# GEOS-ESM/QuickChem

Hardware: AMD Instinct MI355X
Metric: OH gridcells/sec (XGBoost predict), C360 L72 batch (higher is better)
Workload: dtype f32

## Files before the change

### include/ohxgb.h

```cpp
#ifndef OHXGB_H_
#define OHXGB_H_

#include <stdint.h>

#ifdef __cplusplus
extern "C" {
#endif

typedef void* DMatrixHandle;
typedef void* BoosterHandle;
typedef uint64_t bst_ulong;


const char* XGBGetLastError(void);

int XGDMatrixCreateFromMat(const float* data, bst_ulong nrow, bst_ulong ncol, float missing, DMatrixHandle* out);

int XGDMatrixFree(DMatrixHandle handle);

int XGDMatrixNumRow(DMatrixHandle handle, bst_ulong* out);
int XGDMatrixNumCol(DMatrixHandle handle, bst_ulong* out);

int XGDMatrixSaveBinary(DMatrixHandle handle, const char* fname, int silent);
int XGDMatrixCreateFromFile(const char* fname, int silent, DMatrixHandle* out);
// ... 73 lines not shown
  float *ndwet;
  int32_t *k1, *k2;
  float *diag_pl_bst, *diag_tauclwdn, *diag_tauclidn, *diag_taucliup, *diag_tauclwup;
  float *diag_aodup, *diag_aoddn, *diag_aod, *diag_strato3;
} OHXRun1Args;

int OHXBoosterRun1(BoosterHandle handle, const OHXRun1Args* args);
int OHXBoosterRun1Device(BoosterHandle handle, const OHXRun1Args* args, void* stream);

int OHXOHPostProcess(int im, int jm, int km, float avogad, float runiv, float epsilon, const float* ple_mod,
                     const float* t_mod, const float* q_mod, const float* tropp_mod, const float* default_oh,
                     const float* oh_ml, float* oh, float* ndwet);
int OHXOHPostProcessDevice(int im, int jm, int km, float avogad, float runiv, float epsilon, const float* d_ple_mod,
                           const float* d_t_mod, const float* d_q_mod, const float* d_tropp_mod,
                           const float* d_default_oh, const float* d_oh_ml, float* d_oh, float* d_ndwet, void* stream);

int OHXJulianDay(int nymd, int* jday);
int OHXSolarGeometry(int jday, const float* lats, const float* lons, int im, int jm, float degrees_to_radians,
                     float radians_to_degrees, float* lat_deg, float* sza_noon);
int OHXSolarGeometryDevice(int jday, const float* d_lats, const float* d_lons, int im, int jm, float degrees_to_radians,
                           float radians_to_degrees, float* d_lat_deg, float* d_sza_noon, void* stream);

int OHXBoosterGetInfo(BoosterHandle handle, bst_ulong info[8]);
int OHXBoosterGetNumGroups(BoosterHandle handle, bst_ulong* out);
int OHXBoosterGetNumCategoricalSplits(BoosterHandle handle, bst_ulong* out);
int OHXBoosterKernelSymbol(BoosterHandle handle, bst_ulong ncol, const char** out);
int OHXBoosterKernelSymbolRows(BoosterHandle handle, DMatrixHandle dmat, const char** out);
int OHXBoosterRingReruns(BoosterHandle handle, void* stream, bst_ulong* out);
int OHXBoosterCopyEngineChoice(BoosterHandle handle, int* choice, unsigned* trials, unsigned* picked_dma);

typedef void* OHXCommHandle;
#define OHX_UNIQUE_ID_BYTES 128
int OHXCommGetUniqueId(void* id);
int OHXCommInitRank(const void* id, int nranks, int rank, OHXCommHandle* out);
int OHXCommFree(OHXCommHandle comm);
int OHXCommInfo(int* rccl_version);
int OHXShardRows(bst_ulong nrows_total, int nranks, int rank, bst_ulong* row0, bst_ulong* nrows);
int OHXAllGatherOH(OHXCommHandle comm, const float* d_shard, bst_ulong nrows_local, bst_ulong nrows_total,
                   float* d_full, void* stream);

int OHXUnregisterHost(const void* array);

int OHXReleaseScratch(void);

#ifdef __cplusplus
}
// ... 3 lines not shown
```

### quickchem_amd/capi.py

```python
from __future__ import annotations

import ctypes as C
import os
from typing import Optional, Sequence

import numpy as np

_HERE = os.path.dirname(os.path.abspath(__file__))
LIB_PATH = os.path.join(_HERE, "lib", "libohxgb.so")
RING_ROUNDS_DEFAULT = 64
RING_ROUNDS_NO_GRID = 16
RING_ROUNDS_PERMUTED = 4

ABI_SYMBOLS = [
    "XGBGetLastError", "XGDMatrixCreateFromMat", "XGDMatrixFree", "XGDMatrixNumRow", "XGDMatrixNumCol",
    "XGDMatrixSaveBinary", "XGDMatrixCreateFromFile", "XGBoosterCreate", "XGBoosterFree", "XGBoosterLoadModel",
    "XGBoosterSaveModel", "XGBoosterLoadModelFromBuffer", "XGBoosterPredict", "XGBoosterSetParam",
    "OHXDeviceCount", "OHXDMatrixCreateFromDevice", "OHXDMatrixSetGrid", "OHXDMatrixGetGrid", "OHXDMatrixInferGrid", "OHXBoosterPredictDevice", "OHXBoosterCheck",
    "OHXBoosterPredictContribs", "OHXBoosterPredictContribsDevice",
    "OHXBoosterPredictInteractions", "OHXBoosterPredictInteractionsDevice",
    "OHXBoosterPredictContribsFields", "OHXBoosterPredictContribsFieldsDevice",
    "OHXBoosterPredictFields", "OHXBoosterPredictFieldsDevice", "OHXBoosterRun1", "OHXBoosterRun1Device", "OHXOHPostProcess", "OHXOHPostProcessDevice",
    "OHXJulianDay", "OHXSolarGeometry", "OHXSolarGeometryDevice", "OHXBoosterGetInfo", "OHXBoosterGetNumGroups", "OHXBoosterGetNumCategoricalSplits", "OHXBoosterKernelSymbol", "OHXBoosterKernelSymbolRows",
    "OHXBoosterRingReruns", "OHXBoosterCopyEngineChoice", "OHXUnregisterHost", "OHXReleaseScratch",
    "OHXCommGetUniqueId", "OHXCommInitRank", "OHXCommFree", "OHXCommInfo", "OHXShardRows", "OHXAllGatherOH",
]
REFERENCE_BOUND_SYMBOLS = [
    "XGBoosterLoadModel", "XGBoosterSaveModel", "XGDMatrixSaveBinary", "XGDMatrixFree", "XGDMatrixCreateFromFile",
    "XGBoosterPredict", "XGBoosterCreate", "XGDMatrixCreateFromMat", "XGDMatrixNumRow", "XGDMatrixNumCol",
    "XGBoosterFree",
]


class OhxError(RuntimeError):
    pass


class OHXRun1Args(C.Structure):
    _P = C.c_void_p
    _fields_ = ([("im", C.c_int32), ("jm", C.c_int32), ("km", C.c_int32), ("dynamic_k_range", C.c_int32),
                 ("tropp_min", C.c_float), ("ohscale", C.c_float), ("missing", C.c_float),
                 ("avogad", C.c_float), ("runiv", C.c_float), ("epsilon", C.c_float)] +
                [(n, C.c_void_p) for n in ("ple_mod", "t_mod", "q_mod", "tropp_mod", "ple_bst", "zle_bst", "tauclw",
                                           "taucli")] +
                [("scacoef", C.c_void_p * 7)] +
                [(n, C.c_void_p) for n in ("gmito3", "gmitto3", "lat_deg", "t_bst", "no2", "o3", "ch4", "co", "isop",
# ... 51 lines not shown
    lib.OHXDMatrixInferGrid.argtypes = [vp, vp, C.POINTER(i32)]
    lib.OHXBoosterPredictDevice.argtypes = [vp, vp, i32, C.c_uint, vp, vp]
    lib.OHXBoosterCheck.argtypes = [vp, vp]
    lib.OHXBoosterPredictContribs.argtypes = [vp, vp, i32, C.c_uint, C.POINTER(u64), C.POINTER(C.POINTER(f32))]
    lib.OHXBoosterPredictContribsDevice.argtypes = [vp, vp, i32, C.c_uint, vp, vp]
    lib.OHXBoosterPredictInteractions.argtypes = [vp, vp, i32, C.c_uint, C.POINTER(u64), C.POINTER(C.POINTER(f32))]
    lib.OHXBoosterPredictInteractionsDevice.argtypes = [vp, vp, i32, C.c_uint, vp, vp]
    lib.OHXBoosterPredictContribsFields.argtypes = [vp, C.POINTER(vp), C.POINTER(C.c_int32), i32, i32, i32, i32, i32,
                                                    i32, i32, f32, i32, C.c_uint, C.POINTER(vp)]
    lib.OHXBoosterPredictContribsFieldsDevice.argtypes = [vp, C.POINTER(vp), C.POINTER(C.c_int32), i32, i32, i32, i32,
                                                          i32, i32, i32, f32, i32, C.c_uint, C.POINTER(vp), vp]
    lib.OHXBoosterPredictFields.argtypes = [vp, C.POINTER(vp), C.POINTER(C.c_int32), i32, i32, i32, i32, i32, i32, i32,
                                            f32, i32, f32, vp, vp]
    lib.OHXBoosterPredictFieldsDevice.argtypes = [vp, C.POINTER(vp), C.POINTER(C.c_int32), i32, i32, i32, i32, i32,
                                                  i32, i32, f32, i32, f32, vp, vp, vp]
    lib.OHXBoosterRun1.argtypes = [vp, C.POINTER(OHXRun1Args)]
    lib.OHXBoosterRun1Device.argtypes = [vp, C.POINTER(OHXRun1Args), vp]
    lib.OHXOHPostProcess.argtypes = [i32, i32, i32, f32, f32, f32] + [vp] * 8
    lib.OHXOHPostProcessDevice.argtypes = [i32, i32, i32, f32, f32, f32] + [vp] * 9
    lib.OHXJulianDay.argtypes = [i32, C.POINTER(i32)]
    lib.OHXSolarGeometry.argtypes = [i32, vp, vp, i32, i32, f32, f32, vp, vp]
    lib.OHXSolarGeometryDevice.argtypes = [i32, vp, vp, i32, i32, f32, f32, vp, vp, vp]
    lib.OHXBoosterGetInfo.argtypes = [vp, C.POINTER(u64)]
    lib.OHXBoosterGetNumGroups.argtypes = [vp, C.POINTER(u64)]
    lib.OHXBoosterGetNumCategoricalSplits.argtypes = [vp, C.POINTER(u64)]
    lib.OHXBoosterKernelSymbol.argtypes = [vp, u64, C.POINTER(C.c_char_p)]
    lib.OHXBoosterKernelSymbolRows.argtypes = [vp, vp, C.POINTER(C.c_char_p)]
    lib.OHXBoosterRingReruns.argtypes = [vp, vp, C.POINTER(u64)]
    lib.OHXBoosterCopyEngineChoice.argtypes = [vp, C.POINTER(C.c_int), C.POINTER(C.c_uint), C.POINTER(C.c_uint)]
    lib.OHXUnregisterHost.argtypes = [vp]
    lib.OHXReleaseScratch.argtypes = []
    lib.OHXCommGetUniqueId.argtypes = [vp]
    lib.OHXCommInitRank.argtypes = [vp, i32, i32, C.POINTER(vp)]
    lib.OHXCommFree.argtypes = [vp]
    lib.OHXCommInfo.argtypes = [C.POINTER(i32)]
    lib.OHXShardRows.argtypes = [u64, i32, i32, C.POINTER(u64), C.POINTER(u64)]
    lib.OHXAllGatherOH.argtypes = [vp, vp, u64, u64, vp, vp]
    if path == LIB_PATH:
        _lib = lib
    return lib


def check(lib: C.CDLL, rc: int) -> None:
    if rc != 0:
        raise OhxError(lib.XGBGetLastError().decode("utf-8", "replace"))

# ... 269 lines not shown
        if want_diag:
            for name in RUN1_DIAG_3D:
                diag[name] = np.zeros(im * jm * km, dtype=np.float32)
                setattr(args, name, diag[name].ctypes.data)
            diag["diag_strato3"] = np.zeros(im * jm, dtype=np.float32)
            args.diag_strato3 = diag["diag_strato3"].ctypes.data
        return {"args": args, "keep": keep, "oh": oh, "boost": boost, "ndwet": ndwet, "k1": k1, "k2": k2, "diag": diag,
                "shape": (im, jm, km)}

    def run1_call(self, call: dict) -> dict:
        im, jm, km = call["shape"]
        check(self.lib, self.lib.OHXBoosterRun1(self.handle, C.byref(call["args"])))
        unflat = lambda a: None if a is None else a.reshape(km, jm, im).transpose(2, 1, 0)
        out = {"oh": unflat(call["oh"]), "oh_boost": unflat(call["boost"]), "ndwet": unflat(call["ndwet"]),
               "k1": call["k1"].value, "k2": call["k2"].value}
        for name, a in call["diag"].items():
            out[name] = a.reshape(jm, im).T if name == "diag_strato3" else unflat(a)
        return out

    def run1(self, state: dict, **kw) -> dict:
        return self.run1_call(self.run1_prepare(state, **kw))

    def info(self) -> dict:
        arr = (C.c_uint64 * 8)()
        check(self.lib, self.lib.OHXBoosterGetInfo(self.handle, arr))
        keys = ["num_trees", "num_nodes", "num_slots", "node_bytes", "max_depth", "num_feature", "packed",
                "gathers_per_wave"]
        return {k: int(arr[i]) for i, k in enumerate(keys)}

    def ring_reruns(self, stream: int = 0) -> int:
        out = C.c_uint64()
        check(self.lib, self.lib.OHXBoosterRingReruns(self.handle, stream, C.byref(out)))
        return int(out.value)

    def copy_engine_choice(self):
        c, t, d = C.c_int(), C.c_uint(), C.c_uint()
        check(self.lib, self.lib.OHXBoosterCopyEngineChoice(self.handle, C.byref(c), C.byref(t), C.byref(d)))
        return int(c.value), int(t.value), int(d.value)

    def kernel_symbol(self, ncol: int) -> str:
        out = C.c_char_p()
        check(self.lib, self.lib.OHXBoosterKernelSymbol(self.handle, ncol, C.byref(out)))
        return out.value.decode()

    def kernel_symbols_for(self, dmat) -> str:
        out = C.c_char_p()
        check(self.lib, self.lib.OHXBoosterKernelSymbolRows(self.handle, dmat.handle, C.byref(out)))
        return out.value.decode()

    def fields_kernel_symbol(self, nrow: int = 1 << 30) -> str:
# ... 87 lines not shown
```

### quickchem_amd/csrc/capi.cpp

```cpp
#include <hip/hip_runtime_api.h>

#include <algorithm>
#include <cmath>
#include <cstdio>
#include <cstdlib>
#include <cstring>
#include <fstream>
#include <memory>
#include <atomic>
#include <chrono>
#include <mutex>
#include <unordered_map>
#include <sstream>
#include <string>
#include <unordered_set>
#include <vector>

#include "../../include/ohxgb.h"
#include "categorical.hpp"
#include "contribs.hpp"
#include "flatten.hpp"
#include "forest.hpp"
#include "groups.hpp"
#include "kernels.hpp"
// ... 465 lines not shown
  ~BoosterObj() {
    for (hipEvent_t e : {run1_fork, run1_slab, run1_join, run1_clear})
      if (e) (void)hipEventDestroy(e);
    for (hipEvent_t e : run1_prep) (void)hipEventDestroy(e);
    for (hipEvent_t e : run1_walk) (void)hipEventDestroy(e);
    for (hipEvent_t e : run1_feed_events) (void)hipEventDestroy(e);
    if (train.side) (void)hipStreamDestroy(train.side);
    if (train.fork) (void)hipEventDestroy(train.fork);
    if (train.join) (void)hipEventDestroy(train.join);
    if (cluster_done) (void)hipEventDestroy(cluster_done);
    if (defer_seen) (void)hipEventDestroy(defer_seen);
  }
  TrainStreams train;
  Forest forest;
  uint32_t num_groups = 1;
  Forest grouped;
  std::vector<uint32_t> group_begin;
  std::vector<uint32_t> flat_file_index;
  const Forest& flat() const { return num_groups >= 2 ? grouped : forest; }
  bool loaded = false;
  float margin_base = 0.0f;
  std::string margin_error;
  LayoutParams layout;
  std::string kernel_name = "auto";
  int device_pref = -1;
  LaunchTuning tune;
  bool uploaded = false;
  DeviceInfo dev;
  Placement placement;
  bool packed_ok = false;
  DevBuf<PackedNode> d_packed;
  DevBuf<WideNode> d_wide;
  DevBuf<SuperNode> d_super;
  DevBuf<SuperTreeHead> d_super_heads;
  bool super_ok = false;
  uint64_t super_slots = 0;
  uint64_t super_gathers[3] = {0, 0, 0};
  double super_mean_steps = 0.0;
  std::string symbol;
  DevBuf<uint32_t> d_roots;
  DevBuf<uint32_t> d_flags;
  uint32_t ring_reruns_seen = 0;
  DevBuf<float> d_leaves;
  DevBuf<uint32_t> d_defer;
  PinnedBuf<uint32_t> h_defer_count;
  PinnedBuf<uint32_t> h_flags;
  hipEvent_t defer_seen = nullptr;
  bool defer_pending = false;
  uint64_t defer_last_nrow = 0;
  bool defer_too_many = false;
  DevBuf<float> d_pred;
  PinnedBuf<float> h_pred;
  DevBuf<float> d_planes, d_gleaf;
  DevBuf<uint32_t> d_flat_of_file;
  hipStream_t s_copy = nullptr, s_exec = nullptr;
  hipEvent_t run1_fork = nullptr, run1_slab = nullptr, run1_join = nullptr, run1_clear = nullptr;
  std::vector<hipEvent_t> run1_prep, run1_walk, run1_feed_events;
  struct CopyEngineTrial {
    size_t vol = 0;
// ... 129 lines not shown

void ensure_uploaded(BoosterObj& b) {
  if (!b.loaded) throw OhxError("the booster holds no model: call XGBoosterLoadModel first");
  if (b.uploaded) {
    HIP_CHECK(hipSetDevice(b.dev.ordinal));
    return;
  }
  b.dev = use_device(b.device_pref);
  const Forest& flat = b.flat();
  b.placement = place_forest(flat, b.layout);
  b.packed_ok = packed_format_fits(flat, b.placement);
  b.d_roots.upload(b.placement.roots);
  if (b.num_cat != 0) {
    CatForest cf = emit_cat(flat, b.placement);
    b.cat_word_count = cf.words.size();
    b.cat_inline_sets = cf.inline_sets;
    b.cat_word_sets = cf.word_sets;
    if (cf.words.empty()) cf.words.push_back(0u);
    b.d_cat_nodes.upload(cf.nodes);
    b.d_cat_words.upload(cf.words);
    b.d_cat_orig.upload(cf.orig_id);
  } else if (wants_super(b.kernel_name)) {
    SuperForest sf;
    b.super_ok = emit_super(flat, &sf) && sf.nodes.size() * sizeof(SuperNode) < 0xFFFFFFF0ull;
    if (b.super_ok) {
      b.super_slots = sf.nodes.size();
      b.super_gathers[0] = count_super_gathers(sf, 0);
      b.super_gathers[1] = count_super_gathers(sf, 1);
      b.super_gathers[2] = count_super_gathers(sf, 2);
      b.super_mean_steps = mean_super_steps(sf);
      b.d_super.upload(sf.nodes);
      b.d_super_heads.upload(sf.heads);
    }
  }
  if (b.num_cat == 0 && b.packed_ok && !(b.super_ok && wants_super(b.kernel_name))) {
    std::vector<PackedNode> packed = emit_packed(flat, b.placement, nullptr);
    b.d_packed.upload(packed);
  }
  if (b.num_cat == 0 && pick_kernel(b) == KernelKind::Wide) ensure_wide(b);
  b.d_flags.ensure(3);
  {
    LibStreams& ls = lib_streams(b.dev.ordinal);
    b.s_exec = ls.exec;
    b.s_copy = ls.copy;
  }
  HIP_CHECK(hipMemsetAsync(b.d_flags.p, 0, 3 * sizeof(uint32_t), b.s_exec));
  HIP_CHECK(hipStreamSynchronize(b.s_exec));
  b.ring_reruns_seen = 0;
  ensure_train_stream(b);
  b.uploaded = true;
}

void ensure_train_stream(BoosterObj& b) {
  b.tune.train = nullptr;
// ... 1024 lines not shown
  }
  if (n == "ohx_register_host" && handle == nullptr) {
    g_host_registry.on.store(atoi(value) != 0);
    if (atoi(value) == 0) g_host_registry.release_all();
    return 0;
  }
  BoosterObj* b = as_booster(handle);
  if (n == "ohx_kernel") {
    if (v != "auto" && v != "wide" && v != "packed1" && v != "packed2" && v != "packed4" && v != "super1" &&
        v != "super2" && v != "super3" && v != "super4" && v != "ring")
      throw OhxError("ohx_kernel must be one of auto, wide, packed1, packed2, packed4, super1 .. super4, ring");
    if (v != b->kernel_name) invalidate_device_state(*b);
    b->kernel_name = v;
  } else if (n == "ohx_top_levels") {
    int k = atoi(value);
    if (k < 1 || k > 30) throw OhxError("ohx_top_levels must be in 1..30");
    if (k != b->layout.top_levels) invalidate_device_state(*b);
    b->layout.top_levels = k;
  } else if (n == "ohx_line_slots") {
    int k = atoi(value);
    if (k < 0 || k > 1024 || (k & 1)) throw OhxError("ohx_line_slots must be even, 0..1024");
    if (k != b->layout.line_slots) invalidate_device_state(*b);
    b->layout.line_slots = k;
  } else if (n == "ohx_min_chunk") {
    int k = atoi(value);
    if (k < 2 || k > 1024) throw OhxError("ohx_min_chunk must be in 2..1024");
    if (k != b->layout.min_chunk) invalidate_device_state(*b);
    b->layout.min_chunk = k;
  } else if (n == "ohx_launches_per_residency") {
    int k = atoi(value);
    if (k < 0 || k > 1000000) throw OhxError("ohx_launches_per_residency must be >= 0");
    b->tune.launches_per_residency = k;
  } else if (n == "ohx_brick") {
    int e[3] = {-1, -1, -1}, lg[3] = {0, 0, 0};
    if (v == "auto") {
      b->tune.brick_li = b->tune.brick_lj = b->tune.brick_lk = -1;
    } else if (sscanf(value, "%d,%d,%d", &e[0], &e[1], &e[2]) != 3) {
      throw OhxError("ohx_brick must be \"bi,bj,bk\" or \"auto\"");
    } else if (e[0] == 0 && e[1] == 0 && e[2] == 0) {
      b->tune.brick_li = b->tune.brick_lj = b->tune.brick_lk = 0;
    } else {
      for (int q = 0; q < 3; ++q) {
        if (e[q] < 1 || e[q] > 64 || (e[q] & (e[q] - 1))) throw OhxError("ohx_brick extents must be powers of two");
        while ((1 << lg[q]) < e[q]) ++lg[q];
      }
      if (lg[0] + lg[1] + lg[2] != 6) throw OhxError("ohx_brick extents must multiply to 64");
// ... 1019 lines not shown
  b->h_flags.ensure(2);
  void* flags_there = nullptr;
  if (hipHostGetDevicePointer(&flags_there, b->h_flags.p, 0) != hipSuccess) {
    (void)hipGetLastError();
    flags_there = nullptr;
  }
  const bool flags_ride = flags_there != nullptr && back.ride(flags_there, b->d_flags.p, 2);
  back.go();
  TICK_MARK("all-enqueued");
  if (flags_ride) {
    HIP_CHECK(hipStreamSynchronize(main));
    const uint32_t flags[2] = {b->h_flags.p[0], b->h_flags.p[1]};
    judge_flags(*b, flags, main);
  } else {
    raise_flag_errors(*b, main);
  }
  TICK_MARK("done");
  if (trying) b->copy_trial.report(feed.all_by_dma, std::chrono::duration<double>(std::chrono::steady_clock::now() - tick_began).count());
  if (g_tick_trace) g_tick_trace->print(tick);
  g_tick_trace = nullptr;
  API_END();
}

int OHXBoosterGetInfo(BoosterHandle handle, bst_ulong info[8]) {
  API_BEGIN();
  BoosterObj* b = as_booster(handle);
  if (info == nullptr) throw OhxError("OHXBoosterGetInfo: info is NULL");
  if (!b->loaded) throw OhxError("the booster holds no model");
  if (b->num_cat != 0) {
    Placement lp = b->uploaded ? Placement() : place_forest(b->forest, b->layout);
    const Placement& pl = b->uploaded ? b->placement : lp;
    uint64_t words = b->cat_word_count;
    if (!b->uploaded) words = emit_cat(b->forest, pl).words.size();
    info[0] = b->forest.trees.size();
    info[1] = pl.real_nodes;
    info[2] = pl.num_slots;
    info[3] = pl.num_slots * sizeof(CatNode) + words * sizeof(uint32_t);
    info[4] = (bst_ulong)pl.max_depth;
    info[5] = b->forest.num_feature;
    info[6] = 3;
    info[7] = 0;
    return 0;
  }
  Placement local;
  const Placement* p = &b->placement;
  bool packed_ok = b->packed_ok;
  if (!b->uploaded) {
    local = place_forest(b->forest, b->layout);
    p = &local;
    packed_ok = packed_format_fits(b->forest, local);
  }
  const bool packed_used = packed_ok && b->kernel_name != "wide";
  bool super_used = false;
  uint64_t super_slots = b->super_slots;
  auto walk_mode = [&](double mean_steps) {
    const bool ring = b->kernel_name == "ring" ||
                      (b->kernel_name == "auto" && b->forest.num_feature == 27 && mean_steps >= kRingMinMeanSteps);
    return ring ? 2 : (use_tree_tops(b->tune, mean_steps) ? 1 : 0);
  };
  uint64_t super_gathers = b->super_gathers[walk_mode(b->super_mean_steps)];
  if (wants_super(b->kernel_name)) {
    if (b->uploaded) {
      super_used = b->super_ok;
    } else {
      SuperForest sf;
      super_used = emit_super(b->forest, &sf);
      super_slots = sf.nodes.size();
      super_gathers = count_super_gathers(sf, walk_mode(mean_super_steps(sf)));
    }
  }
  info[0] = b->forest.trees.size();
  info[1] = p->real_nodes;
  info[2] = super_used ? super_slots : p->num_slots;
  info[3] = super_used ? super_slots * sizeof(SuperNode)
                       : p->num_slots * (packed_used ? sizeof(PackedNode) : sizeof(WideNode));
  info[4] = (bst_ulong)p->max_depth;
  info[5] = b->forest.num_feature;
  info[6] = super_used ? 2 : (packed_used ? 1 : 0);
  info[7] = super_used ? super_gathers : 0;
  API_END();
}

int OHXBoosterGetNumGroups(BoosterHandle handle, bst_ulong* out) {
  API_BEGIN();
  BoosterObj* b = as_booster(handle);
  if (out == nullptr) throw OhxError("OHXBoosterGetNumGroups: out is NULL");
  if (!b->loaded) throw OhxError("the booster holds no model: call XGBoosterLoadModel first");
  *out = b->num_groups;
  API_END();
}

int OHXBoosterGetNumCategoricalSplits(BoosterHandle handle, bst_ulong* out) {
  API_BEGIN();
  BoosterObj* b = as_booster(handle);
  if (out == nullptr) throw OhxError("OHXBoosterGetNumCategoricalSplits: out is NULL");
  if (!b->loaded) throw OhxError("the booster holds no model: call XGBoosterLoadModel first");
  *out = b->num_cat;
  API_END();
}

int OHXBoosterKernelSymbol(BoosterHandle handle, bst_ulong ncol, const char** out) {
  API_BEGIN();
  BoosterObj* b = as_booster(handle);
// ... 85 lines not shown
```

### quickchem_amd/csrc/flatten.cpp

```cpp
#include "flatten.hpp"

#include <limits>

#include <algorithm>
#include <cmath>
#include <cstring>
#include <deque>

namespace ohx {

namespace {

struct Pair {
  int32_t l, r;
  int depth;
};

}

Placement place_forest(const Forest& f, const LayoutParams& lp) {
  Placement p;
  p.layout = lp;
  const int line = lp.line_slots;
  if (line != 0 && (line < 2 || (line & 1))) throw OhxError("layout: line_slots must be even and >= 2");
// ... 100 lines not shown
}

namespace {

int choose_super_phase(const Tree& t) {
  double cost[2] = {0.0, 0.0};
  bool have_cover = false;
  for (float h : t.sum_hess) have_cover = have_cover || h > 0.0f;
  std::vector<std::pair<int32_t, int>> stack{{0, 0}};
  while (!stack.empty()) {
    auto [n, d] = stack.back();
    stack.pop_back();
    if (t.left[(size_t)n] == -1) {
      const double w = have_cover ? (double)t.sum_hess[(size_t)n] : 1.0;
      cost[d & 1] += w;
    } else {
      stack.emplace_back(t.left[(size_t)n], d + 1);
      stack.emplace_back(t.right[(size_t)n], d + 1);
    }
  }
  return cost[1] < cost[0] ? 1 : 0;
}

}

bool emit_super(const Forest& f, SuperForest* out) {
  out->nodes.clear();
  out->heads.clear();
  if (f.num_feature > kSuperLeaf) return false;
  const float inf = std::numeric_limits<float>::infinity();
  const SuperNode unused{inf, inf, inf, super_meta(0, 0, 0, 1, 1, 1, 0)};
  const uint32_t leaf_meta = super_meta(kSuperLeaf, kSuperLeaf, kSuperLeaf, 0, 0, 0, 0);
  struct Item {
    int32_t node;
    uint32_t slot;
    uint32_t level;
  };
  std::vector<Item> queue;
  for (const Tree& t : f.trees) {
    const uint32_t base = (uint32_t)out->nodes.size();
    SuperTreeHead head{base, 0u, 0.0f, 0u};
    std::vector<SuperNode> sn(8, unused);
    uint32_t next_group = 2;
    queue.clear();
    const bool root_is_leaf = t.left[0] == -1;
    const int phase = root_is_leaf ? 0 : choose_super_phase(t);
    if (phase == 1) {
      head.root_meta = (t.feature[0] & 31u) | ((uint32_t)(t.default_left[0] ? 1u : 0u) << 5) | (1u << 8);
      head.root_thr = t.value[0];
      queue.push_back({t.left[0], 4u, 0u});
      queue.push_back({t.right[0], 5u, 0u});
    } else {
      queue.push_back({0, 4u, 0u});
    }
    for (size_t qi = 0; qi < queue.size(); ++qi) {
      const Item it = queue[qi];
      const size_t n = (size_t)it.node;
      SuperNode s = unused;
      if (t.left[n] == -1) {
        s.thr0 = s.thrL = s.thrR = t.value[n];
        s.meta = leaf_meta;
      } else {
        const size_t l = (size_t)t.left[n], r = (size_t)t.right[n];
        const bool l_int = t.left[l] != -1, r_int = t.left[r] != -1;
        s.thr0 = t.value[n];
        s.thrL = t.value[l];
        s.thrR = t.value[r];
        uint32_t meta = super_meta(t.feature[n], l_int ? t.feature[l] : kSuperLeaf, r_int ? t.feature[r] : kSuperLeaf,
                                   t.default_left[n] ? 1u : 0u, (l_int && t.default_left[l]) ? 1u : 0u,
                                   (r_int && t.default_left[r]) ? 1u : 0u, 0u);
        if (l_int || r_int) {
          const uint32_t grp = next_group++;
          if (grp >= kSuperMaxGroups) {
            out->nodes.clear();
            out->heads.clear();
            return false;
          }
          meta |= grp << 18;
          sn.resize((size_t)next_group * 4, unused);
          if (l_int) {
            queue.push_back({t.left[l], grp * 4 + 0, it.level + 1});
            queue.push_back({t.right[l], grp * 4 + 1, it.level + 1});
          }
          if (r_int) {
            queue.push_back({t.left[r], grp * 4 + 2, it.level + 1});
            queue.push_back({t.right[r], grp * 4 + 3, it.level + 1});
          }
        }
        s.meta = meta;
      }
      if (it.level <= 2 && it.slot >= kSuperTopSlots) throw OhxError("internal error: tree top outside its first records");
      if (it.level <= 3 && it.slot >= kSuperRingSlots) throw OhxError("internal error: a record of the first four steps outside the tree's first 176");
      sn[it.slot] = s;
      if (it.level + 1 > head.steps) head.steps = it.level + 1;
    }
    out->heads.push_back(head);
    out->nodes.insert(out->nodes.end(), sn.begin(), sn.end());
    if (out->nodes.size() >= 0xFFFFFFF0ull) throw OhxError("booster too large for the super-node format");
  }
  out->nodes.insert(out->nodes.end(), kSuperTopSlots, unused);
  return true;
}

Forest group_major(const Forest& f, std::vector<uint32_t>* group_begin, std::vector<uint32_t>* file_index) {
  const uint32_t G = f.num_groups();
  group_begin->assign((size_t)G + 1, 0u);
  for (int32_t g : f.tree_info) ++(*group_begin)[(size_t)g + 1];
  for (uint32_t g = 0; g < G; ++g) (*group_begin)[g + 1] += (*group_begin)[g];
  std::vector<uint32_t> next(group_begin->begin(), group_begin->end() - 1);
  file_index->assign(f.trees.size(), 0u);
  for (size_t t = 0; t < f.trees.size(); ++t) (*file_index)[next[(size_t)f.tree_info[t]]++] = (uint32_t)t;
  Forest out;
  out.base_score = f.base_score;
  out.num_feature = f.num_feature;
  out.num_class = f.num_class;
  out.num_target = f.num_target;
  out.major_version = f.major_version;
// ... 94 lines not shown
```

### quickchem_amd/csrc/flatten.hpp

```cpp
#pragma once
#include <cstdint>
#include <vector>

#include "forest.hpp"

namespace ohx {

struct LayoutParams {
  int top_levels = 9;
  int line_slots = 16;
  int min_chunk = 6;
};

struct PackedNode {
  uint32_t value_bits;
  uint32_t meta;
};

struct WideNode {
  float value;
  uint32_t left;
  uint32_t feat_dl;
  int32_t orig_id;
};
// ... 14 lines not shown
struct SuperNode {
  float thr0, thrL, thrR;
  uint32_t meta;
};
constexpr uint32_t kSuperLeaf = 31u;
constexpr uint32_t super_meta(uint32_t f0, uint32_t fl, uint32_t fr, uint32_t dl0, uint32_t dll, uint32_t dlr,
                              uint32_t group) {
  return (fl & 31u) | (dl0 << 5) | (dll << 6) | (dlr << 7) | ((f0 & 31u) << 8) | ((fr & 31u) << 13) | (group << 18);
}
constexpr uint32_t kSuperMaxGroups = 1u << 14;
constexpr uint32_t kSuperTopSlots = 48;
constexpr uint32_t kSuperRingSlots = 176;

struct SuperTreeHead {
  uint32_t base;
  uint32_t root_meta;
  float root_thr;
  uint32_t steps;
};

struct SuperForest {
  std::vector<SuperNode> nodes;
  std::vector<SuperTreeHead> heads;
};

Forest group_major(const Forest& f, std::vector<uint32_t>* group_begin, std::vector<uint32_t>* file_index);

struct CatNode {
  uint32_t bits;
  uint32_t left;
  uint32_t meta;
  float size;
};
static_assert(sizeof(CatNode) == 16, "one 128-bit load per node");
constexpr uint32_t kCatFlag = 1u << 30;
constexpr uint32_t kCatWords = 1u << 29;
constexpr uint32_t kCatFeatureMask = kCatWords - 1u;

struct CatForest {
  std::vector<CatNode> nodes;
  std::vector<uint32_t> words;
  std::vector<int32_t> orig_id;
  uint64_t inline_sets = 0, word_sets = 0;
};
CatForest emit_cat(const Forest& f, const Placement& p);

bool emit_super(const Forest& f, SuperForest* out);

Placement place_forest(const Forest& f, const LayoutParams& lp);
bool packed_format_fits(const Forest& f, const Placement& p);
std::vector<PackedNode> emit_packed(const Forest& f, const Placement& p, std::vector<int32_t>* orig_id);
std::vector<WideNode> emit_wide(const Forest& f, const Placement& p);

}
```

### quickchem_amd/csrc/synth_host.cpp

```cpp
#include <algorithm>
#include <cmath>
#ifdef _OPENMP
#include <omp.h>
#endif
#include <cstdint>
#include <cstdlib>
#include <cstring>
#include <deque>
#include <string>
#include <vector>

#include "flatten.hpp"
#include "forest.hpp"
#include "synth_common.h"

using namespace ohx;

namespace {

thread_local std::string g_err;

struct Work {
  int32_t node;
  uint32_t lo, hi;
// ... 196 lines not shown

int ohx_model_convert(const uint8_t* in_buf, uint64_t in_len, int format, uint8_t** out_buf, uint64_t* out_len) {
  try {
    Forest f = load_model_buffer(in_buf, (size_t)in_len);
    f.validate();
    if (format == 1) {
      std::string s = write_json_model(f);
      *out_buf = (uint8_t*)malloc(s.size());
      memcpy(*out_buf, s.data(), s.size());
      *out_len = s.size();
    } else {
      std::vector<uint8_t> b = format == 2 ? write_ubjson_model(f) : write_legacy_binary(f);
      *out_buf = (uint8_t*)malloc(b.size());
      memcpy(*out_buf, b.data(), b.size());
      *out_len = b.size();
    }
    return 0;
  } catch (const std::exception& e) {
    g_err = e.what();
    return -1;
  }
}

int ohx_super_walk_cpu(const uint8_t* model, uint64_t model_len, const float* rows, uint64_t nrow, uint32_t ncol,
                       float missing, float* out, uint64_t* info) {
  try {
    Forest f = load_model_buffer(model, (size_t)model_len);
    f.validate();
    SuperForest sf;
    if (!emit_super(f, &sf)) return 1;
    uint64_t phase1 = 0, steps = 0;
    for (const SuperTreeHead& h : sf.heads) {
      phase1 += (h.root_meta >> 8) & 1u;
      steps += h.steps;
    }
    if (info) {
      info[0] = sf.nodes.size();
      info[1] = phase1;
      info[2] = steps;
    }
    const bool missing_is_nan = missing != missing;
    std::vector<float> x(32, 0.0f);
    for (uint64_t r = 0; r < nrow; ++r) {
      for (uint32_t c = 0; c < 32; ++c) {
        float v = c < ncol ? rows[r * ncol + c] : (c < f.num_feature ? NAN : 0.0f);
        if (c < ncol && !missing_is_nan && v == missing) v = NAN;
        x[c] = v;
      }
      float acc = f.base_score;
      for (const SuperTreeHead& h : sf.heads) {
        auto left = [](float xv, float thr, bool dl) { return xv != xv ? dl : xv < thr; };
        uint32_t rel = 4u;
        if (h.root_meta & 0x100u) rel += left(x[h.root_meta & 31u], h.root_thr, (h.root_meta & 32u) != 0) ? 0u : 1u;
// ... 8 lines not shown
          const float thr1 = l0 ? s.thrL : s.thrR;
          const uint32_t f1 = (w >> (l0 ? 0u : 13u)) & 31u;
          if (f1 == 31u) {
            memcpy(&leaf_bits, &thr1, 4);
            ++taken;
          }
          const bool l1 = left(x[f1], thr1, ((w >> (l0 ? 6u : 7u)) & 1u) != 0);
          rel = ((w >> 18) << 2) + (l0 ? 0u : 2u) + (l1 ? 0u : 1u);
        }
        if (taken != 1) throw OhxError("a walk must meet exactly one leaf code, met " + std::to_string(taken));
        float leaf;
        memcpy(&leaf, &leaf_bits, 4);
        acc += leaf;
      }
      out[r] = acc;
    }
    return 0;
  } catch (const std::exception& e) {
    g_err = e.what();
    return -1;
  }
}

int ohx_super_heads_cpu(const uint8_t* model, uint64_t model_len, uint32_t* out, uint64_t cap, uint64_t* ntrees) {
  try {
    Forest f = load_model_buffer(model, (size_t)model_len);
    f.validate();
    SuperForest sf;
    if (!emit_super(f, &sf)) return 1;
    *ntrees = sf.heads.size();
    for (size_t t = 0; t < sf.heads.size() && t < cap; ++t) {
      out[2 * t] = (sf.heads[t].root_meta >> 8) & 1u;
      out[2 * t + 1] = sf.heads[t].steps;
    }
    return 0;
  } catch (const std::exception& e) {
    g_err = e.what();
    return -1;
  }
}

int ohx_cat_flatten_cpu(const uint8_t* model, uint64_t model_len, uint32_t* nodes, uint64_t cap_slots, uint32_t* words,
                        uint64_t cap_words, int32_t* orig_id, uint32_t* roots, uint64_t cap_trees, uint64_t* info) {
  try {
    Forest f = load_model_buffer(model, (size_t)model_len);
    f.validate();
// ... 23 lines not shown
```

### quickchem_amd/synth.py

```python
from __future__ import annotations

import ctypes as C
import os
from dataclasses import dataclass
from typing import Dict, Tuple

import numpy as np

from . import capi

_HERE = os.path.dirname(os.path.abspath(__file__))
SYNTH_LIB_PATH = os.path.join(_HERE, "lib", "libohx_synth.so")
SYNTH_GPU_LIB_PATH = os.path.join(_HERE, "lib", "libohx_synth_gpu.so")

FEATURE_SEED = 20241108
MODEL_SEED = 1060
NFEAT = 27
FEATURE_NAMES = ["LAT", "PL", "T", "NO2", "O3", "CH4", "CO", "ISOP", "ACET", "C2H6", "C3H8",
                 "PRPE", "ALK4", "MP", "H2O2", "TAUCLWDN", "TAUCLIDN", "TAUCLIUP", "TAUCLWUP",
                 "CLOUD", "QV", "GMISTRATO3", "ALBUV", "AODUP", "AODDN", "CH2O", "SZA"]
IS2D = [n in ("LAT", "GMISTRATO3", "ALBUV", "SZA") for n in FEATURE_NAMES]
PL_FEATURE = 1
XX_MISS = -999.0

# ... 8 lines not shown
}

_lib = None


def _load():
    global _lib
    if _lib is None:
        if not os.path.exists(SYNTH_LIB_PATH):
            raise capi.OhxError(f"{SYNTH_LIB_PATH} is missing: run __graft_entry__.build()")
        lib = C.CDLL(SYNTH_LIB_PATH)
        lib.ohx_synth_last_error.restype = C.c_char_p
        lib.ohx_synth_rows_cpu.argtypes = [C.c_uint32, C.c_int, C.c_int, C.c_int, C.c_uint64, C.c_uint64, C.c_void_p]
        lib.ohx_synth_field_cpu.argtypes = [C.c_uint32, C.c_int, C.c_int, C.c_int, C.c_int, C.c_void_p]
        lib.ohx_synth_model.argtypes = [C.c_uint32, C.c_int, C.c_int, C.c_int, C.c_int, C.c_uint32, C.c_int, C.c_int,
                                        C.c_int, C.c_float, C.c_float, C.c_int, C.POINTER(C.c_void_p),
                                        C.POINTER(C.c_uint64), C.POINTER(C.c_uint64)]
        lib.ohx_synth_free.argtypes = [C.c_void_p]
        lib.ohx_synth_set_threads.argtypes = [C.c_int]
        lib.ohx_model_convert.argtypes = [C.c_void_p, C.c_uint64, C.c_int, C.POINTER(C.c_void_p),
                                          C.POINTER(C.c_uint64)]
        lib.ohx_super_walk_cpu.argtypes = [C.c_void_p, C.c_uint64, C.c_void_p, C.c_uint64, C.c_uint32, C.c_float,
                                           C.c_void_p, C.POINTER(C.c_uint64)]
        lib.ohx_super_heads_cpu.argtypes = [C.c_void_p, C.c_uint64, C.c_void_p, C.c_uint64, C.POINTER(C.c_uint64)]
        lib.ohx_contribs_cpu.argtypes = [C.c_void_p, C.c_uint64, C.c_void_p, C.c_uint64, C.c_uint64, C.c_float, C.c_int,
                                         C.c_uint, C.c_void_p]
        lib.ohx_contribs_table_stats.argtypes = [C.c_void_p, C.c_uint64, C.POINTER(C.c_uint64)]
        lib.ohx_contribs_plan.argtypes = [C.c_uint64, C.c_uint32, C.c_uint32, C.c_int, C.POINTER(C.c_uint64)]
        lib.ohx_interactions_cpu.argtypes = [C.c_void_p, C.c_uint64, C.c_void_p, C.c_uint64, C.c_uint64, C.c_float,
                                             C.c_int, C.c_uint, C.c_void_p]
        lib.ohx_interactions_table_stats.argtypes = [C.c_void_p, C.c_uint64, C.POINTER(C.c_uint64)]
        lib.ohx_interactions_plan.argtypes = [C.c_uint64, C.c_uint32, C.c_uint32, C.c_int, C.POINTER(C.c_uint64)]
        lib.ohx_cat_flatten_cpu.argtypes = [C.c_void_p, C.c_uint64, C.c_void_p, C.c_uint64, C.c_void_p, C.c_uint64,
                                            C.c_void_p, C.c_void_p, C.c_uint64, C.POINTER(C.c_uint64)]
        _lib = lib
    return _lib


def set_threads(n: int) -> None:
    _load().ohx_synth_set_threads(int(n))


def _check(rc: int) -> None:
    if rc != 0:
        raise capi.OhxError(_load().ohx_synth_last_error().decode())

# ... 50 lines not shown
    src = np.frombuffer(bytes(image), dtype=np.uint8) if not isinstance(image, np.ndarray) else image
    out, n = C.c_void_p(), C.c_uint64()
    code = {"binary": 0, "json": 1, "ubj": 2}[fmt]
    _check(lib.ohx_model_convert(src.ctypes.data, src.nbytes, code, C.byref(out), C.byref(n)))
    return _take(out, n.value)


def cat_flatten_cpu(image):
    lib = _load()
    src = np.frombuffer(bytes(image), dtype=np.uint8) if not isinstance(image, np.ndarray) else image
    info = (C.c_uint64 * 5)()
    _check(lib.ohx_cat_flatten_cpu(src.ctypes.data, src.nbytes, None, 0, None, 0, None, None, 0, info))
    slots, nwords, ntrees = int(info[0]), int(info[1]), int(info[2])
    nodes = np.zeros((slots, 4), dtype=np.uint32)
    words = np.zeros(max(nwords, 1), dtype=np.uint32)
    orig_id = np.zeros(slots, dtype=np.int32)
    roots = np.zeros(ntrees, dtype=np.uint32)
    _check(lib.ohx_cat_flatten_cpu(src.ctypes.data, src.nbytes, nodes.ctypes.data, slots, words.ctypes.data, nwords,
                                   orig_id.ctypes.data, roots.ctypes.data, ntrees, info))
    return {"nodes": nodes, "words": words[:nwords], "orig_id": orig_id, "roots": roots,
            "inline_sets": int(info[3]), "word_sets": int(info[4])}


def super_walk_cpu(image, rows: np.ndarray, missing: float = XX_MISS):
    lib = _load()
    src = np.frombuffer(bytes(image), dtype=np.uint8) if not isinstance(image, np.ndarray) else image
    rows = np.ascontiguousarray(rows, dtype=np.float32)
    out = np.empty(rows.shape[0], dtype=np.float32)
    info = (C.c_uint64 * 4)()
    rc = lib.ohx_super_walk_cpu(src.ctypes.data, src.nbytes, rows.ctypes.data, rows.shape[0], rows.shape[1], missing,
                                out.ctypes.data, info)
    if rc == 1:
        return None, None
    _check(rc)
    return out, {"super_nodes": int(info[0]), "phase1_trees": int(info[1]), "steps": int(info[2])}


def super_heads_cpu(image):
    lib = _load()
    src = np.frombuffer(bytes(image), dtype=np.uint8) if not isinstance(image, np.ndarray) else image
    n = C.c_uint64()
    rc = lib.ohx_super_heads_cpu(src.ctypes.data, src.nbytes, None, 0, C.byref(n))
    if rc == 1:
        return None
    _check(rc)
    out = np.zeros((n.value, 2), dtype=np.uint32)
    _check(lib.ohx_super_heads_cpu(src.ctypes.data, src.nbytes, out.ctypes.data, n.value, C.byref(n)))
    return out


def contribs_cpu(image, rows: np.ndarray, num_feature: int, missing: float = XX_MISS, approximate: bool = False,
                 ntree_limit: int = 0) -> np.ndarray:
    lib = _load()
    src = np.frombuffer(bytes(image), dtype=np.uint8) if not isinstance(image, np.ndarray) else image
    rows = np.ascontiguousarray(rows, dtype=np.float32)
    out = np.empty((rows.shape[0], num_feature + 1), dtype=np.float32)
    _check(lib.ohx_contribs_cpu(src.ctypes.data, src.nbytes, rows.ctypes.data, rows.shape[0], rows.shape[1], missing,
                                1 if approximate else 0, ntree_limit, out.ctypes.data))
# ... 114 lines not shown
```

Measured before the change: 2.426 billion.

## Pair sibling super-node groups into shared 128-byte lines

Renumbers the super-node groups of each tree so that the two child groups reached from adjacent records sit side by side in one 128-byte line. Each tree is padded to start on a line boundary, and a lone group at the same level fills an odd slot where one is available. The aim is that the gathers in the super-node tree walk touch fewer distinct cache lines. The cost is extra pad records and a larger node array, and trees that would exceed the group limit keep the old layout; new info counters report pad records and fallback trees.

```diff
diff --git a/include/ohxgb.h b/include/ohxgb.h
--- a/include/ohxgb.h
+++ b/include/ohxgb.h
@@ -119,6 +119,7 @@
                            float radians_to_degrees, float* d_lat_deg, float* d_sza_noon, void* stream);
 
 int OHXBoosterGetInfo(BoosterHandle handle, bst_ulong info[8]);
+int OHXBoosterGetInfoEx(BoosterHandle handle, bst_ulong n, bst_ulong* info);
 int OHXBoosterGetNumGroups(BoosterHandle handle, bst_ulong* out);
 int OHXBoosterGetNumCategoricalSplits(BoosterHandle handle, bst_ulong* out);
 int OHXBoosterKernelSymbol(BoosterHandle handle, bst_ulong ncol, const char** out);
diff --git a/quickchem_amd/capi.py b/quickchem_amd/capi.py
--- a/quickchem_amd/capi.py
+++ b/quickchem_amd/capi.py
@@ -21,7 +21,7 @@
     "OHXBoosterPredictInteractions", "OHXBoosterPredictInteractionsDevice",
     "OHXBoosterPredictContribsFields", "OHXBoosterPredictContribsFieldsDevice",
     "OHXBoosterPredictFields", "OHXBoosterPredictFieldsDevice", "OHXBoosterRun1", "OHXBoosterRun1Device", "OHXOHPostProcess", "OHXOHPostProcessDevice",
-    "OHXJulianDay", "OHXSolarGeometry", "OHXSolarGeometryDevice", "OHXBoosterGetInfo", "OHXBoosterGetNumGroups", "OHXBoosterGetNumCategoricalSplits", "OHXBoosterKernelSymbol", "OHXBoosterKernelSymbolRows",
+    "OHXJulianDay", "OHXSolarGeometry", "OHXSolarGeometryDevice", "OHXBoosterGetInfo", "OHXBoosterGetInfoEx", "OHXBoosterGetNumGroups", "OHXBoosterGetNumCategoricalSplits", "OHXBoosterKernelSymbol", "OHXBoosterKernelSymbolRows",
     "OHXBoosterRingReruns", "OHXBoosterCopyEngineChoice", "OHXUnregisterHost", "OHXReleaseScratch",
     "OHXCommGetUniqueId", "OHXCommInitRank", "OHXCommFree", "OHXCommInfo", "OHXShardRows", "OHXAllGatherOH",
 ]
@@ -119,6 +119,8 @@
     lib.OHXSolarGeometry.argtypes = [i32, vp, vp, i32, i32, f32, f32, vp, vp]
     lib.OHXSolarGeometryDevice.argtypes = [i32, vp, vp, i32, i32, f32, f32, vp, vp, vp]
     lib.OHXBoosterGetInfo.argtypes = [vp, C.POINTER(u64)]
+    if hasattr(lib, "OHXBoosterGetInfoEx"):
+        lib.OHXBoosterGetInfoEx.argtypes = [vp, u64, C.POINTER(u64)]
     lib.OHXBoosterGetNumGroups.argtypes = [vp, C.POINTER(u64)]
     lib.OHXBoosterGetNumCategoricalSplits.argtypes = [vp, C.POINTER(u64)]
     lib.OHXBoosterKernelSymbol.argtypes = [vp, u64, C.POINTER(C.c_char_p)]
@@ -434,10 +436,13 @@
         return self.run1_call(self.run1_prepare(state, **kw))
 
     def info(self) -> dict:
-        arr = (C.c_uint64 * 8)()
-        check(self.lib, self.lib.OHXBoosterGetInfo(self.handle, arr))
         keys = ["num_trees", "num_nodes", "num_slots", "node_bytes", "max_depth", "num_feature", "packed",
-                "gathers_per_wave"]
+                "gathers_per_wave", "pad_records", "fallback_trees"]
+        arr = (C.c_uint64 * len(keys))()
+        if hasattr(self.lib, "OHXBoosterGetInfoEx"):
+            check(self.lib, self.lib.OHXBoosterGetInfoEx(self.handle, len(keys), arr))
+        else:
+            check(self.lib, self.lib.OHXBoosterGetInfo(self.handle, arr))
         return {k: int(arr[i]) for i, k in enumerate(keys)}
 
     def ring_reruns(self, stream: int = 0) -> int:
diff --git a/quickchem_amd/csrc/capi.cpp b/quickchem_amd/csrc/capi.cpp
--- a/quickchem_amd/csrc/capi.cpp
+++ b/quickchem_amd/csrc/capi.cpp
@@ -511,6 +511,7 @@
   float margin_base = 0.0f;
   std::string margin_error;
   LayoutParams layout;
+  bool pair_lines = true;
   std::string kernel_name = "auto";
   int device_pref = -1;
   LaunchTuning tune;
@@ -524,6 +525,8 @@
   DevBuf<SuperTreeHead> d_super_heads;
   bool super_ok = false;
   uint64_t super_slots = 0;
+  uint64_t super_pad_records = 0;
+  uint64_t super_fallback_trees = 0;
   uint64_t super_gathers[3] = {0, 0, 0};
   double super_mean_steps = 0.0;
   std::string symbol;
@@ -699,14 +702,18 @@
     b.d_cat_orig.upload(cf.orig_id);
   } else if (wants_super(b.kernel_name)) {
     SuperForest sf;
-    b.super_ok = emit_super(flat, &sf) && sf.nodes.size() * sizeof(SuperNode) < 0xFFFFFFF0ull;
+    b.super_ok = emit_super(flat, &sf, b.pair_lines) && sf.nodes.size() * sizeof(SuperNode) < 0xFFFFFFF0ull;
     if (b.super_ok) {
       b.super_slots = sf.nodes.size();
+      b.super_pad_records = sf.pad_records;
+      b.super_fallback_trees = sf.fallback_trees;
       b.super_gathers[0] = count_super_gathers(sf, 0);
       b.super_gathers[1] = count_super_gathers(sf, 1);
       b.super_gathers[2] = count_super_gathers(sf, 2);
       b.super_mean_steps = mean_super_steps(sf);
       b.d_super.upload(sf.nodes);
+      if (b.pair_lines && ((uintptr_t)b.d_super.p & 127u) != 0)
+        throw OhxError("internal error: the super-node array is not aligned to a 128-byte line");
       b.d_super_heads.upload(sf.heads);
     }
   }
@@ -1777,6 +1784,13 @@
     if (k < 0 || k > 1024 || (k & 1)) throw OhxError("ohx_line_slots must be even, 0..1024");
     if (k != b->layout.line_slots) invalidate_device_state(*b);
     b->layout.line_slots = k;
+  } else if (n == "ohx_pair_lines") {
+    bool on;
+    if (v == "on" || v == "1") on = true;
+    else if (v == "off" || v == "0") on = false;
+    else throw OhxError("ohx_pair_lines must be on or off");
+    if (on != b->pair_lines) invalidate_device_state(*b);
+    b->pair_lines = on;
   } else if (n == "ohx_min_chunk") {
     int k = atoi(value);
     if (k < 2 || k > 1024) throw OhxError("ohx_min_chunk must be in 2..1024");
@@ -2842,11 +2856,32 @@
   API_END();
 }
 
+constexpr int kInfoEntries = 10;
+static void booster_info(BoosterObj* b, bst_ulong info[kInfoEntries]);
+
 int OHXBoosterGetInfo(BoosterHandle handle, bst_ulong info[8]) {
   API_BEGIN();
   BoosterObj* b = as_booster(handle);
   if (info == nullptr) throw OhxError("OHXBoosterGetInfo: info is NULL");
+  bst_ulong all[kInfoEntries];
+  booster_info(b, all);
+  std::copy(all, all + 8, info);
+  API_END();
+}
+
+int OHXBoosterGetInfoEx(BoosterHandle handle, bst_ulong n, bst_ulong* info) {
+  API_BEGIN();
+  BoosterObj* b = as_booster(handle);
+  if (info == nullptr) throw OhxError("OHXBoosterGetInfoEx: info is NULL");
+  bst_ulong all[kInfoEntries];
+  booster_info(b, all);
+  for (bst_ulong i = 0; i < n; ++i) info[i] = i < (bst_ulong)kInfoEntries ? all[i] : 0;
+  API_END();
+}
+
+static void booster_info(BoosterObj* b, bst_ulong info[kInfoEntries]) {
   if (!b->loaded) throw OhxError("the booster holds no model");
+  info[8] = info[9] = 0;
   if (b->num_cat != 0) {
     Placement lp = b->uploaded ? Placement() : place_forest(b->forest, b->layout);
     const Placement& pl = b->uploaded ? b->placement : lp;
@@ -2860,7 +2895,7 @@
     info[5] = b->forest.num_feature;
     info[6] = 3;
     info[7] = 0;
-    return 0;
+    return;
   }
   Placement local;
   const Placement* p = &b->placement;
@@ -2872,7 +2907,7 @@
   }
   const bool packed_used = packed_ok && b->kernel_name != "wide";
   bool super_used = false;
-  uint64_t super_slots = b->super_slots;
+  uint64_t super_slots = b->super_slots, pad_records = b->super_pad_records, fallback_trees = b->super_fallback_trees;
   auto walk_mode = [&](double mean_steps) {
     const bool ring = b->kernel_name == "ring" ||
                       (b->kernel_name == "auto" && b->forest.num_feature == 27 && mean_steps >= kRingMinMeanSteps);
@@ -2884,8 +2919,10 @@
       super_used = b->super_ok;
     } else {
       SuperForest sf;
-      super_used = emit_super(b->forest, &sf);
+      super_used = emit_super(b->forest, &sf, b->pair_lines);
       super_slots = sf.nodes.size();
+      pad_records = sf.pad_records;
+      fallback_trees = sf.fallback_trees;
       super_gathers = count_super_gathers(sf, walk_mode(mean_super_steps(sf)));
     }
   }
@@ -2898,7 +2935,8 @@
   info[5] = b->forest.num_feature;
   info[6] = super_used ? 2 : (packed_used ? 1 : 0);
   info[7] = super_used ? super_gathers : 0;
-  API_END();
+  info[8] = super_used ? pad_records : 0;
+  info[9] = super_used ? fallback_trees : 0;
 }
 
 int OHXBoosterGetNumGroups(BoosterHandle handle, bst_ulong* out) {
diff --git a/quickchem_amd/csrc/flatten.cpp b/quickchem_amd/csrc/flatten.cpp
--- a/quickchem_amd/csrc/flatten.cpp
+++ b/quickchem_amd/csrc/flatten.cpp
@@ -146,11 +146,62 @@
   return cost[1] < cost[0] ? 1 : 0;
 }
 
-}
-
-bool emit_super(const Forest& f, SuperForest* out) {
+bool pair_super_lines(std::vector<SuperNode>* sn, const std::vector<uint32_t>& level, const SuperNode& unused) {
+  const uint32_t ngroups = (uint32_t)(sn->size() / 4);
+  auto child = [&](uint32_t rec) { return (*sn)[rec].meta >> 18; };
+  uint32_t frozen = std::min(ngroups, 2u);
+  for (uint32_t rec = 0; rec < std::min<uint32_t>((uint32_t)sn->size(), kSuperRingSlots); ++rec)
+    frozen = std::max(frozen, child(rec) + 1u);
+  if (frozen >= ngroups) return true;
+  struct Unit {
+    uint32_t a, b;
+  };
+  std::vector<Unit> units;
+  for (uint32_t rec = 0; rec + 1 < (uint32_t)sn->size(); rec += 2) {
+    uint32_t a = child(rec), b = child(rec + 1);
+    if (a < frozen) a = 0;
+    if (b < frozen) b = 0;
+    if (a && b) units.push_back({a, b});
+    else if (a || b) units.push_back({a | b, 0u});
+  }
+  std::vector<uint32_t> new_of(ngroups, 0u);
+  for (uint32_t g = 0; g < frozen; ++g) new_of[g] = g;
+  uint32_t next = frozen;
+  size_t lone_from = 0;
+  for (size_t u = 0; u < units.size(); ++u) {
+    const Unit un = units[u];
+    if (un.b == 0) {
+      if (!new_of[un.a]) new_of[un.a] = next++;
+      continue;
+    }
+    if (next & 1u) {
+      lone_from = std::max(lone_from, u + 1);
+      while (lone_from < units.size() && (units[lone_from].b != 0 || new_of[units[lone_from].a] != 0)) ++lone_from;
+      if (lone_from < units.size() && level[units[lone_from].a] == level[un.a]) new_of[units[lone_from].a] = next;
+      ++next;
+    }
+    new_of[un.a] = next++;
+    new_of[un.b] = next++;
+  }
+  if (next >= kSuperMaxGroups) return false;
+  std::vector<SuperNode> paired((size_t)next * 4, unused);
+  for (uint32_t g = 0; g < ngroups; ++g)
+    for (uint32_t j = 0; j < 4; ++j) {
+      SuperNode s = (*sn)[(size_t)g * 4 + j];
+      if ((s.meta >> 18) != 0) s.meta = (s.meta & 0x3FFFFu) | (new_of[s.meta >> 18] << 18);
+      paired[(size_t)new_of[g] * 4 + j] = s;
+    }
+  sn->swap(paired);
+  return true;
+}
+
+}
+
+bool emit_super(const Forest& f, SuperForest* out, bool pair_lines) {
   out->nodes.clear();
   out->heads.clear();
+  out->pad_records = 0;
+  out->fallback_trees = 0;
   if (f.num_feature > kSuperLeaf) return false;
   const float inf = std::numeric_limits<float>::infinity();
   const SuperNode unused{inf, inf, inf, super_meta(0, 0, 0, 1, 1, 1, 0)};
@@ -161,12 +212,14 @@
     uint32_t level;
   };
   std::vector<Item> queue;
+  std::vector<uint32_t> group_level;
   for (const Tree& t : f.trees) {
     const uint32_t base = (uint32_t)out->nodes.size();
     SuperTreeHead head{base, 0u, 0.0f, 0u};
     std::vector<SuperNode> sn(8, unused);
     uint32_t next_group = 2;
     queue.clear();
+    group_level.assign(2, 0u);
     const bool root_is_leaf = t.left[0] == -1;
     const int phase = root_is_leaf ? 0 : choose_super_phase(t);
     if (phase == 1) {
@@ -202,6 +255,7 @@
           }
           meta |= grp << 18;
           sn.resize((size_t)next_group * 4, unused);
+          group_level.push_back(it.level + 1);
           if (l_int) {
             queue.push_back({t.left[l], grp * 4 + 0, it.level + 1});
             queue.push_back({t.right[l], grp * 4 + 1, it.level + 1});
@@ -217,6 +271,13 @@
       if (it.level <= 3 && it.slot >= kSuperRingSlots) throw OhxError("internal error: a record of the first four steps outside the tree's first 176");
       sn[it.slot] = s;
       if (it.level + 1 > head.steps) head.steps = it.level + 1;
+    }
+    if (pair_lines) {
+      const size_t plain = sn.size();
+      if (!pair_super_lines(&sn, group_level, unused)) ++out->fallback_trees;
+      if (sn.size() & 4u) sn.insert(sn.end(), 4, unused);
+      out->pad_records += sn.size() - plain;
+      if (base % 8u != 0) throw OhxError("internal error: a tree of the paired layout does not start on a 128-byte line");
     }
     out->heads.push_back(head);
     out->nodes.insert(out->nodes.end(), sn.begin(), sn.end());
diff --git a/quickchem_amd/csrc/flatten.hpp b/quickchem_amd/csrc/flatten.hpp
--- a/quickchem_amd/csrc/flatten.hpp
+++ b/quickchem_amd/csrc/flatten.hpp
@@ -60,7 +60,11 @@
 struct SuperForest {
   std::vector<SuperNode> nodes;
   std::vector<SuperTreeHead> heads;
+  uint64_t pad_records = 0;
+  uint32_t fallback_trees = 0;
 };
+
+constexpr uint32_t kSuperFrozenGroups = kSuperRingSlots / 4;
 
 Forest group_major(const Forest& f, std::vector<uint32_t>* group_begin, std::vector<uint32_t>* file_index);
 
@@ -83,7 +87,7 @@
 };
 CatForest emit_cat(const Forest& f, const Placement& p);
 
-bool emit_super(const Forest& f, SuperForest* out);
+bool emit_super(const Forest& f, SuperForest* out, bool pair_lines = true);
 
 Placement place_forest(const Forest& f, const LayoutParams& lp);
 bool packed_format_fits(const Forest& f, const Placement& p);
diff --git a/quickchem_amd/csrc/synth_host.cpp b/quickchem_amd/csrc/synth_host.cpp
--- a/quickchem_amd/csrc/synth_host.cpp
+++ b/quickchem_amd/csrc/synth_host.cpp
@@ -242,13 +242,13 @@
   }
 }
 
-int ohx_super_walk_cpu(const uint8_t* model, uint64_t model_len, const float* rows, uint64_t nrow, uint32_t ncol,
-                       float missing, float* out, uint64_t* info) {
+int ohx_super_walk_layout_cpu(const uint8_t* model, uint64_t model_len, const float* rows, uint64_t nrow, uint32_t ncol,
+                              float missing, int pair_lines, float* out, uint64_t* info) {
   try {
     Forest f = load_model_buffer(model, (size_t)model_len);
     f.validate();
     SuperForest sf;
-    if (!emit_super(f, &sf)) return 1;
+    if (!emit_super(f, &sf, pair_lines != 0)) return 1;
     uint64_t phase1 = 0, steps = 0;
     for (const SuperTreeHead& h : sf.heads) {
       phase1 += (h.root_meta >> 8) & 1u;
@@ -303,6 +303,32 @@
   }
 }
 
+int ohx_super_walk_cpu(const uint8_t* model, uint64_t model_len, const float* rows, uint64_t nrow, uint32_t ncol,
+                       float missing, float* out, uint64_t* info) {
+  return ohx_super_walk_layout_cpu(model, model_len, rows, nrow, ncol, missing, 1, out, info);
+}
+
+int ohx_super_flatten_cpu(const uint8_t* model, uint64_t model_len, int pair_lines, uint32_t* nodes, uint64_t cap_nodes,
+                          uint32_t* heads, uint64_t cap_trees, uint64_t* info) {
+  try {
+    Forest f = load_model_buffer(model, (size_t)model_len);
+    f.validate();
+    SuperForest sf;
+    if (!emit_super(f, &sf, pair_lines != 0)) return 1;
+    info[0] = sf.nodes.size();
+    info[1] = sf.heads.size();
+    info[2] = sf.pad_records;
+    info[3] = sf.fallback_trees;
+    static_assert(sizeof(SuperNode) == 16 && sizeof(SuperTreeHead) == 16, "four words each");
+    if (cap_nodes) memcpy(nodes, sf.nodes.data(), 16 * (size_t)std::min<uint64_t>(cap_nodes, sf.nodes.size()));
+    if (cap_trees) memcpy(heads, sf.heads.data(), 16 * (size_t)std::min<uint64_t>(cap_trees, sf.heads.size()));
+    return 0;
+  } catch (const std::exception& e) {
+    g_err = e.what();
+    return -1;
+  }
+}
+
 int ohx_super_heads_cpu(const uint8_t* model, uint64_t model_len, uint32_t* out, uint64_t cap, uint64_t* ntrees) {
   try {
     Forest f = load_model_buffer(model, (size_t)model_len);
diff --git a/quickchem_amd/synth.py b/quickchem_amd/synth.py
--- a/quickchem_amd/synth.py
+++ b/quickchem_amd/synth.py
@@ -54,6 +54,10 @@
                                           C.POINTER(C.c_uint64)]
         lib.ohx_super_walk_cpu.argtypes = [C.c_void_p, C.c_uint64, C.c_void_p, C.c_uint64, C.c_uint32, C.c_float,
                                            C.c_void_p, C.POINTER(C.c_uint64)]
+        lib.ohx_super_walk_layout_cpu.argtypes = [C.c_void_p, C.c_uint64, C.c_void_p, C.c_uint64, C.c_uint32, C.c_float,
+                                                  C.c_int, C.c_void_p, C.POINTER(C.c_uint64)]
+        lib.ohx_super_flatten_cpu.argtypes = [C.c_void_p, C.c_uint64, C.c_int, C.c_void_p, C.c_uint64, C.c_void_p,
+                                              C.c_uint64, C.POINTER(C.c_uint64)]
         lib.ohx_super_heads_cpu.argtypes = [C.c_void_p, C.c_uint64, C.c_void_p, C.c_uint64, C.POINTER(C.c_uint64)]
         lib.ohx_contribs_cpu.argtypes = [C.c_void_p, C.c_uint64, C.c_void_p, C.c_uint64, C.c_uint64, C.c_float, C.c_int,
                                          C.c_uint, C.c_void_p]
@@ -150,18 +154,33 @@
             "inline_sets": int(info[3]), "word_sets": int(info[4])}
 
 
-def super_walk_cpu(image, rows: np.ndarray, missing: float = XX_MISS):
+def super_walk_cpu(image, rows: np.ndarray, missing: float = XX_MISS, pair_lines: bool = True):
     lib = _load()
     src = np.frombuffer(bytes(image), dtype=np.uint8) if not isinstance(image, np.ndarray) else image
     rows = np.ascontiguousarray(rows, dtype=np.float32)
     out = np.empty(rows.shape[0], dtype=np.float32)
     info = (C.c_uint64 * 4)()
-    rc = lib.ohx_super_walk_cpu(src.ctypes.data, src.nbytes, rows.ctypes.data, rows.shape[0], rows.shape[1], missing,
-                                out.ctypes.data, info)
+    rc = lib.ohx_super_walk_layout_cpu(src.ctypes.data, src.nbytes, rows.ctypes.data, rows.shape[0], rows.shape[1],
+                                       missing, 1 if pair_lines else 0, out.ctypes.data, info)
     if rc == 1:
         return None, None
     _check(rc)
     return out, {"super_nodes": int(info[0]), "phase1_trees": int(info[1]), "steps": int(info[2])}
+
+
+def super_flatten_cpu(image, pair_lines: bool = True):
+    lib = _load()
+    src = np.frombuffer(bytes(image), dtype=np.uint8) if not isinstance(image, np.ndarray) else image
+    info = (C.c_uint64 * 4)()
+    rc = lib.ohx_super_flatten_cpu(src.ctypes.data, src.nbytes, 1 if pair_lines else 0, None, 0, None, 0, info)
+    if rc == 1:
+        return None
+    _check(rc)
+    nodes = np.zeros((int(info[0]), 4), dtype=np.uint32)
+    heads = np.zeros((int(info[1]), 4), dtype=np.uint32)
+    _check(lib.ohx_super_flatten_cpu(src.ctypes.data, src.nbytes, 1 if pair_lines else 0, nodes.ctypes.data,
+                                     nodes.shape[0], heads.ctypes.data, heads.shape[0], info))
+    return {"nodes": nodes, "heads": heads, "pad_records": int(info[2]), "fallback_trees": int(info[3])}
 
 
 def super_heads_cpu(image):
```

After: 2.450 billion, median of 6. No clear change (+1.0%).
